# Hxyou/MSCLIP

Hardware: AMD Instinct MI355X
Metric: image-text pairs/sec ViT-B/32 bf16 (higher is better)
Workload: dtype bf16; 1 GPU; MS-CLIP-S b32-yfcc-msclips fwd + contrastive step (both towers, gather, logits, symmetric CE), per-GPU batch 512, 224x224 images + 77-token captions, random-init weights; per_gpu_batch=512, global_batch=512, parallelism=dp1, bn=eval (folded running statistics), rccl_ranks=1

## Files before the change

msclip_amd/csrc/backward.hip:

```cpp
#include <mutex>
#include <type_traits>
#include <stdlib.h>
#include "common.h"
#include "plan.h"
#include "../../include/msclip_hip.h"
#include "../../include/msclip_ext2.h"

namespace {

__device__ __forceinline__ float sigmoidf_fast(float z) { return 1.f / (1.f + __expf(-z)); }

__global__ __launch_bounds__(256) void transpose_kernel(const bf16_t* __restrict__ in, int ldi, bf16_t* __restrict__ out,
                                                        int ldo, int M, int C, int Mpad) {
  __shared__ bf16_t tile[64][66];
  const int m0 = blockIdx.x * 64, c0 = blockIdx.y * 64;
  const int tx = threadIdx.x & 63, ty = threadIdx.x >> 6;
  for (int r = ty; r < 64; r += 4) {
    const int m = m0 + r, c = c0 + tx;
    tile[r][tx] = (m < M && c < C) ? in[(size_t)m * ldi + c] : (bf16_t)0;
  }
  __syncthreads();
  for (int r = ty; r < 64; r += 4) {
    const int c = c0 + r, m = m0 + tx;
    if (c < C && m < Mpad) out[(size_t)c * ldo + m] = tile[tx][r];
// ... 678 lines not shown
                                                int part_blocks, int skip_group, const float* row_scale, void* stream) {
  MSCLIP_PLAN_HOOK(msclip_cast_bf16_colsum_rowscale, stream, x, ldx, y, ldy, M, C, part, part_blocks, skip_group, row_scale);
  return cast_bf16_colsum_launch(x, ldx, y, ldy, M, C, part, part_blocks, skip_group, row_scale, stream);
}

extern "C" int msclip_ext2_abi_version(void) { return MSCLIP_EXT2_ABI_VERSION; }

static bool colsum_two_stage() {
  static int v = -1;
  if (v < 0) {
    const char* e = getenv("MSCLIP_COLSUM_TWO_STAGE");
    v = e && e[0] == '1';
  }
  return v != 0;
}
static unsigned* colsum_counters(int n) {
  constexpr int RING = 1 << 18, MAXDEV = 16;
  static unsigned* ring[MAXDEV] = {};
  static int next[MAXDEV] = {};
  static std::mutex mu;
  int dev = 0;
  if (hipGetDevice(&dev) != hipSuccess || dev < 0 || dev >= MAXDEV || n > RING) return nullptr;
  std::lock_guard<std::mutex> lock(mu);
  if (!ring[dev]) {
    if (hipMalloc((void**)&ring[dev], RING * sizeof(unsigned)) != hipSuccess) { ring[dev] = nullptr; return nullptr; }
    if (hipMemset(ring[dev], 0, RING * sizeof(unsigned)) != hipSuccess || hipDeviceSynchronize() != hipSuccess) return nullptr;
  }
  if (next[dev] + n > RING) next[dev] = 0;
  unsigned* p = ring[dev] + next[dev];
  next[dev] += n;
  return p;
}

extern "C" int msclip_prepare_device(void) { return colsum_counters(0) ? MSCLIP_OK : MSCLIP_ELAUNCH; }

extern "C" int msclip_colsum(const void* x, int ld, int is_f32, float* out, int M, int N, int accumulate, float* scratch,
                             int chunks, void* stream) {
  MSCLIP_PLAN_HOOK(msclip_colsum, stream, x, ld, is_f32, out, M, N, accumulate, scratch, chunks);
  if (!x || !out || M <= 0 || N <= 0 || ld < N || chunks < 1 || (chunks > 1 && !scratch)) return MSCLIP_EINVAL;
  hipStream_t st = (hipStream_t)stream;
  if (is_f32 && M <= 32 && N >= 16384 && !(N % 4) && !(ld % 4) && !((size_t)x % 16) && !((size_t)out % 16)) {
    hipLaunchKernelGGL(fold_rows_kernel, dim3(grid_for((size_t)N / 4, 256, 8192)), dim3(256), 0, st, (const float*)x, (size_t)ld,
                       out, M, (size_t)N / 4, accumulate);
    return msclip_launch_status();
  }
  const int rpc = (M + chunks - 1) / chunks;
  float* first = chunks > 1 ? scratch : out;
  int cpr = 1;
  while (cpr < 32 && cpr * 8 < N) cpr *= 2;
  const bool wide = !is_f32 && !(N % 8) && !(ld % 8) && !((size_t)x % 16);
  const int colblocks = wide ? (N + cpr * 8 - 1) / (cpr * 8) : (N + 63) / 64;
  unsigned* counters = chunks > 1 && !colsum_two_stage() ? colsum_counters(colblocks) : nullptr;
  if (is_f32)
    hipLaunchKernelGGL(colsum_kernel<float>, dim3(colblocks, chunks), dim3(256), 0, st, (const float*)x, ld, first, M, N,
                       chunks > 1 ? 0 : accumulate, rpc, out, counters, accumulate);
  else if (wide)
    hipLaunchKernelGGL(colsum_bf16x8_kernel, dim3(colblocks, chunks), dim3(256), 0, st, (const bf16_t*)x,
                       ld, first, M, N, chunks > 1 ? 0 : accumulate, rpc, cpr, out, counters, accumulate);
  else
    hipLaunchKernelGGL(colsum_kernel<bf16_t>, dim3(colblocks, chunks), dim3(256), 0, st, (const bf16_t*)x, ld, first, M,
                       N, chunks > 1 ? 0 : accumulate, rpc, out, counters, accumulate);
  if (chunks > 1 && !counters)
    hipLaunchKernelGGL(colsum_kernel<float>, dim3((N + 63) / 64, 1), dim3(256), 0, st, (const float*)scratch, N, out, chunks, N,
                       accumulate, chunks);
  return msclip_launch_status();
}

// ... 124 lines not shown
```

msclip_amd/csrc/gemm.hip:

```cpp
#include <stdlib.h>
#include <type_traits>
#include "common.h"
#include "plan.h"
#include "../../include/msclip_hip.h"
#include "../../include/msclip_ext2.h"
#include "gemm_epilogue.h"

namespace {

constexpr int BK = 64;

struct RowSrc {
  long long pix;
  int ih0, iw0;
  int ok;
};



template <int MODE, int BM, int BN, int WM, int WN, bool RS = false>
__global__ __launch_bounds__(WM * WN * 64, 2) void gemm_kernel(const msclip_gemm_desc a_in) {
  msclip_gemm_desc a = a_in;
  if (MODE == 0 && gridDim.y > 1) {
    const int kc = a.K / (int)gridDim.y;
    a.X = (const bf16_t*)a.X + (size_t)blockIdx.y * kc;
    a.W = (const bf16_t*)a.W + (size_t)blockIdx.y * kc;
    a.out = (float*)a.out + (size_t)blockIdx.y * a.M * a.ldo;
    a.K = kc;
  }
  constexpr int NW = WM * WN;
  constexpr int NT = NW * 64;
  constexpr int TM = BM / WM / 32, TN = BN / WN / 32;
  constexpr int XI = BM * 8 / NT, WI = BN * 8 / NT;
  constexpr int NPC = XI + WI;
// ... 179 lines not shown
    else
      epilogue_generic<TM, TN, RS>(acc, a, vec, cm0 + wm, cn0 + wn, lane);
  }
}


constexpr int PSLOTS = 10, PREG = 128 * 64;
#ifndef PP_NOEPI
#define PP_NOEPI 0
#endif

__device__ __forceinline__ bf16x8 pp_ld(const void* p) { return *(const bf16x8*)p; }

typedef __attribute__((ext_vector_type(8))) int i32x8;
template <bool F8>
__device__ __forceinline__ f32x4 pp_mma(const bf16x8 (&w)[2], const bf16x8 (&x)[2], int ks, f32x4 c) {
  if constexpr (F8) {
    i32x8 a, b;
    __builtin_memcpy(&a, &w[0], 32);
    __builtin_memcpy(&b, &x[0], 32);
    return __builtin_amdgcn_mfma_scale_f32_16x16x128_f8f6f4(a, b, c, 0, 0, 0, 0x7f7f7f7f, 0, 0x7f7f7f7f);
  } else {
    return __builtin_amdgcn_mfma_f32_16x16x32_bf16(w[ks], x[ks], c, 0, 0, 0);
  }
}

typedef __attribute__((ext_vector_type(4))) __bf16 bf16x4v;
__device__ __forceinline__ bf16x8 pp_ld_tr(const char* p) {
  const bf16x4v lo = __builtin_amdgcn_ds_read_tr16_b64_v4bf16((AS3 bf16x4v*)p);
  const bf16x4v hi = __builtin_amdgcn_ds_read_tr16_b64_v4bf16((AS3 bf16x4v*)(p + 1024));
  return __builtin_shufflevector(lo, hi, 0, 1, 2, 3, 4, 5, 6, 7);
}

template <int MODE, bool F8 = false, int EPI = 0, bool TNL = false>
__global__ __launch_bounds__(512) void gemm_pp_kernel(const msclip_gemm_desc a_in, const float* __restrict__ row_scale,
                                                      const float* __restrict__ col_scale) {
  static_assert(!(F8 && MODE == 1), "fp8 operands: dense GEMM only");
  static_assert(EPI == 0 || (MODE == 0 && (!F8 || EPI == 2)), "LayerNorm fold: dense GEMM; fp8 operands as the producer only");
  static_assert(EPI != 3 || !F8, "training dgrad epilogue: bf16 operands");
  static_assert(EPI != 4 || !F8, "row-scaled residual update (msclip_gemm_rowscale; row_scale = its table): bf16 operands");
  static_assert(!TNL || (MODE == 0 && !F8 && EPI == 0), "token-major operands: dense bf16 GEMM, plain epilogues");
  msclip_gemm_desc a = a_in;
  if (a.M_dev) a.M = min(a.M, *a.M_dev);
  unsigned kbase = 0;
  const int ktot = a.K;
  if (TNL) {
    const int kc = ((a.K + 63) / 64 + (int)gridDim.y - 1) / (int)gridDim.y * 64;
    kbase = blockIdx.y * (unsigned)kc;
    a.out = (float*)a.out + (size_t)blockIdx.y * a.M * a.ldo;
    a.K = kc;
  } else
  if (MODE == 0 && !F8 && gridDim.y > 1) {
    const int kc = a.K / (int)gridDim.y;
    a.X = (const bf16_t*)a.X + (size_t)blockIdx.y * kc;
    a.W = (const bf16_t*)a.W + (size_t)blockIdx.y * kc;
    a.out = (float*)a.out + (size_t)blockIdx.y * a.M * a.ldo;
    a.K = kc;
  }
  constexpr unsigned ES = F8 ? 1u : 2u;
  constexpr int KT = F8 ? 128 : 64;
  constexpr int TM = 4, TN = 2;
  constexpr bool TE = MODE == 0 && !F8 && EPI == 0;
  __shared__ __attribute__((aligned(1024))) bf16_t smem[PSLOTS * PREG];

  const int tid = threadIdx.x;
  const int lane = tid & 63;
  const int wave = __builtin_amdgcn_readfirstlane(tid >> 6);
  const int grp = wave >> 2;
  const int nt_n = (a.N + 255) / 256;
  const int nt_m = (a.M + 255) / 256;
  const int ntiles = nt_n * nt_m;
  const int nk = a.K / KT;

  constexpr int CG = 4;
  const unsigned tper = (unsigned)(nt_m * CG);
  const unsigned tper_rcp = 0xffffffffu / tper + 1u;
  const int wg_tail = nt_n - (nt_n - 1) / CG * CG;
  const unsigned wgt_rcp = 0xffffffffu / (unsigned)wg_tail + 1u;
  auto tile_origin = [&](int t, int& m0, int& n0) {
    const int q = ntiles >> 3, r = ntiles & 7, x = t & 7;
    const unsigned id = (unsigned)((x < r ? x * (q + 1) : r * (q + 1) + (x - r) * q) + (t >> 3));
    const unsigned g = (unsigned)(((unsigned long long)id * tper_rcp) >> 32);
    const unsigned idg = id - g * tper;
    const bool tail = (int)(g * CG + CG) > nt_n;
    const unsigned wg = tail ? (unsigned)wg_tail : (unsigned)CG;
    const unsigned row = !tail ? idg >> 2 : wg_tail == 1 ? idg : (unsigned)(((unsigned long long)idg * wgt_rcp) >> 32);
    m0 = (int)(row * 256u);
    n0 = (int)((g * CG + (idg - row * wg)) * 256u);
  };

  unsigned vx[2], vw[2];
#pragma unroll
  for (int i = 0; i < 2; ++i) {
    if (TNL) {
      const int row = (wave + 8 * i) * 4 + (lane >> 4);
      const int g = (row & 3) | (((row >> 3) & 1) << 2);
      const unsigned ch = (unsigned)(((((lane & 15) >> 1) ^ g) << 1) | (lane & 1)) << 4;
      vx[i] = (unsigned)row * (unsigned)a.ldx * 2u + ch;
      vw[i] = (unsigned)row * (unsigned)a.ldw * 2u + ch;
      continue;
    }
    const int row = (wave + 8 * i) * 8 + (lane >> 3);
    const unsigned ch = (unsigned)((lane & 7) ^ ((row >> 1) & 7)) << 4;
    vx[i] = (unsigned)row * (unsigned)a.ldx * ES + ch;
    vw[i] = (unsigned)row * (unsigned)a.ldw * ES + ch;
  }
  const unsigned xhalf = TNL ? 256u : 128u * (unsigned)a.ldx * ES, whalf = TNL ? 256u : 128u * (unsigned)a.ldw * ES;
  int ti = blockIdx.x, kti = 0, islot = 0;
  __amdgpu_buffer_rsrc_t rx, rw;
  int cpix[2][2], chw[2][2];
  int ce = 0;
  auto set_tile = [&](int t) {
    if (MODE == 1) {
      int m0 = 0, n0 = 0;
      if (t < ntiles) tile_origin(t, m0, n0);
      const int hw = a.Ho * a.Wo;
#pragma unroll
      for (int h = 0; h < 2; ++h)
#pragma unroll
        for (int i = 0; i < 2; ++i) {
          const int row = (wave + 8 * i) * 8 + (lane >> 3);
          const int m = m0 + h * 128 + row;
          const int b = m / hw, rem = m - b * hw;
          const int ho = rem / a.Wo, wo = rem - ho * a.Wo;
          const int ih0 = ho * a.stride - a.pad, iw0 = wo * a.stride - a.pad;
          const int ihs = (t < ntiles && m < a.M) ? ih0 : -(1 << 14);
          chw[h][i] = (ihs & 0xffff) | (iw0 << 16);
          cpix[h][i] = (((b * a.H + ih0) * a.Wd + iw0) * a.Cin) * 2 + (((lane & 7) ^ ((row >> 1) & 7)) << 4);
        }
      const unsigned long long wb = (unsigned long long)(a.N - n0) * (unsigned long long)a.ldw * ES;
      rw = t < ntiles ? make_rsrc((const char*)a.W + (size_t)n0 * a.ldw * ES, wb > 0xffffffffull ? 0xffffffffu : (unsigned)wb)
                      : make_rsrc(a.W, 0);
      return;
    }
    if (TNL) {
      int m0 = 0, n0 = 0;
      if (t < ntiles) tile_origin(t, m0, n0);
      const unsigned long long xb = (unsigned long long)ktot * a.ldx * 2ull - (unsigned long long)m0 * 2ull;
      const unsigned long long wb = (unsigned long long)ktot * a.ldw * 2ull - (unsigned long long)n0 * 2ull;
      rx = t < ntiles ? make_rsrc((const char*)a.X + (size_t)m0 * 2, (unsigned)xb) : make_rsrc(a.X, 0);
      rw = t < ntiles ? make_rsrc((const char*)a.W + (size_t)n0 * 2, (unsigned)wb) : make_rsrc(a.W, 0);
// ... 19 lines not shown
    if (TNL) {
      const unsigned kr = kbase + (unsigned)kti * 64u;
      if (J < 2) {
        const unsigned ro = kr * (unsigned)a.ldw * 2u;
        blds16(rw, vw[0] + ro, (J & 1) * 256u, dst);
        blds16(rw, vw[1] + ro, (J & 1) * 256u, dst + 8 * 512);
      } else {
        const unsigned ro = kr * (unsigned)a.ldx * 2u;
        blds16(rx, vx[0] + ro, (J & 1) * 256u, dst);
        blds16(rx, vx[1] + ro, (J & 1) * 256u, dst + 8 * 512);
      }
    } else
    if (J < 2) {
      blds16(rw, vw[0], ko + (J & 1) * whalf, dst);
      blds16(rw, vw[1], ko + (J & 1) * whalf, dst + 8 * 512);
    } else if (MODE == 1) {
      const int kh = (ce >> 20) & 15, kw = (ce >> 24) & 15, doff = (ce & 0xfffff) * 2;
#pragma unroll
      for (int i = 0; i < 2; ++i) {
        const int ih = ((chw[J & 1][i] << 16) >> 16) + kh, iw = (chw[J & 1][i] >> 16) + kw;
        const bool ok = (unsigned)ih < (unsigned)a.H && (unsigned)iw < (unsigned)a.Wd;
        blds16(rx, ok ? (unsigned)(cpix[J & 1][i] + doff) : 0x80000000u, 0, dst + i * 8 * 512);
      }
    } else {
      blds16(rx, vx[0], ko + (J & 1) * xhalf, dst);
      blds16(rx, vx[1], ko + (J & 1) * xhalf, dst + 8 * 512);
    }
    if (MODE == 1 && J == 1) {
      const int* tp = a.ktab + kti * 8;
      asm volatile("s_load_dword %0, %1, 0x0\n\ts_waitcnt lgkmcnt(0)" : "=s"(ce) : "s"(tp));
    }
    islot = islot == PSLOTS - 1 ? 0 : islot + 1;
    if (J == 3) {
      if (++kti == nk) {
        kti = 0;
        ti += gridDim.x;
        set_tile(ti);
      }
    }
  };
  using I0 = std::integral_constant<int, 0>;
  using I1 = std::integral_constant<int, 1>;
  using I2 = std::integral_constant<int, 2>;
  using I3 = std::integral_constant<int, 3>;

  const int wm = grp * 128, wn = (wave & 3) * 64;
  const int r16 = lane & 15, quad = lane >> 4;
  const bool vec = !((a.N | a.ldo | (a.resid_kind ? a.ldr : 0)) & 3);
  const bool plain_rows = a.rpg == 0x7fffffff && a.resid_kind != 3 && a.resid_kind < 5;
  int la[2];
#pragma unroll
  for (int ks = 0; ks < 2; ++ks)
    la[ks] = r16 * 128 + (((F8 ? (quad << 1) | ks : (ks << 2) | quad) ^ ((r16 >> 1) & 7)) << 4);
  const int wsub = ((wave >> 1) & 1);
  const int woff = (wave & 1) * 64 * 128;
  const int lt = (8 * quad + (r16 >> 2)) * 256 + ((((r16 >> 2) & 3) | ((quad & 1) << 2)) << 5) + (r16 & 3) * 8;
  const int ltw = lt ^ ((wave & 1) * 128);
  const char* lds = (const char*)smem;

  if (MODE == 1)
    rx = make_rsrc(a.X, (unsigned)((long long)(a.M / (a.Ho * a.Wo)) * a.H * a.Wd * a.Cin * 2));
  set_tile(ti);
  issue(I0{}); issue(I1{}); issue(I2{}); issue(I3{});
  issue(I0{}); issue(I1{}); issue(I2{});
  issue(I3{});
  asm volatile("s_waitcnt vmcnt(8)" ::: "memory");
  __builtin_amdgcn_s_barrier();
  asm volatile("" ::: "memory");
  if (grp) __builtin_amdgcn_s_barrier();

  int cslot = 0;
  bf16x8 w0[2][2], w1[2][2], xf[4][2];
  int epi_stores = 0;
  for (int tc = blockIdx.x; tc < ntiles; tc += gridDim.x) {
    int cm0, cn0;
    tile_origin(tc, cm0, cn0);
    f32x4 acc[4][8];
#pragma unroll
    for (int i = 0; i < 4; ++i)
#pragma unroll
      for (int j = 0; j < 8; ++j)
#pragma unroll
        for (int r = 0; r < 4; ++r) acc[i][j][r] = 0.f;
    int lane_s;
    asm volatile("v_mbcnt_lo_u32_b32 %0, -1, 0\n\tv_mbcnt_hi_u32_b32 %0, -1, %0" : "=v"(lane_s));
    const bool seg2 = EPI == 1 && a.W2 && cm0 >= a.seg_split;
    const float* bseg = seg2 ? a.bias2 : a.bias;
    const float* bsrc = bseg ? bseg : (const float*)a.zero;
    const int nlast = bseg ? a.N - 1 : 0;
    float bcol;
    {
      const int n = cn0 + wn + lane_s;
      const float* p = bsrc + (n < nlast ? n : nlast);
      asm volatile("global_load_dword %0, %1, off" : "=&v"(bcol) : "v"(p));
    }
    float ccol = 0.f;
    f32x4 rstat4 = {1.f, 0.f, 1.f, 0.f};
    if constexpr (EPI == 1) {
      const float* p = (seg2 ? a.csum2 : a.csum) + cn0 + wn + lane_s;
      asm volatile("global_load_dword %0, %1, off" : "=&v"(ccol) : "v"(p));
      const float* q0 = a.rowstat + 2 * (size_t)(cm0 + wm + lane_s);
      f32x2 lo, hi;
      asm volatile("global_load_dwordx2 %0, %1, off" : "=&v"(lo) : "v"(q0));
      asm volatile("global_load_dwordx2 %0, %1, off offset:512" : "=&v"(hi) : "v"(q0));
      rstat4 = f32x4{lo[0], lo[1], hi[0], hi[1]};
    } else if constexpr (EPI == 2) {
      const float* q0 = a.center + cm0 + wm + lane_s;
      float lo, hi;
      asm volatile("global_load_dword %0, %1, off" : "=&v"(lo) : "v"(q0));
      asm volatile("global_load_dword %0, %1, off offset:256" : "=&v"(hi) : "v"(q0));
      rstat4 = f32x4{lo, 0.f, hi, 0.f};
    }

    float pf_sink = 0.f;
    for (int kt = 0; kt < nk; ++kt) {
      int s1 = cslot + wsub, s2 = cslot + 2 + grp;
      if (s1 >= PSLOTS) s1 -= PSLOTS;
      if (s2 >= PSLOTS) s2 -= PSLOTS;
      const char* wreg = lds + s1 * (PREG * 2) + woff;
      const char* xreg = lds + s2 * (PREG * 2);
      cslot = cslot + 4 >= PSLOTS ? cslot + 4 - PSLOTS : cslot + 4;

#define PP_PRIO(x) __builtin_amdgcn_s_setprio(x)
#define PP_LGK() asm volatile("s_waitcnt lgkmcnt(0)" ::: "memory")
#define PP_SYNC_IN()                                   \
  __builtin_amdgcn_sched_barrier(0);                   \
  __builtin_amdgcn_s_barrier();                        \
  PP_LGK();                                            \
  __builtin_amdgcn_sched_barrier(0);                   \
  PP_PRIO(1)
#define PP_SYNC_OUT()                                  \
  PP_PRIO(0);                                          \
  __builtin_amdgcn_sched_barrier(0);                   \
  __builtin_amdgcn_s_barrier();                        \
  asm volatile("" ::: "memory");                       \
  __builtin_amdgcn_sched_barrier(0)

      const size_t wtn = (size_t)(lds + s1 * (PREG * 2) + ltw), xtn = (size_t)(lds + s2 * (PREG * 2) + lt);
      if constexpr (TNL) {
#pragma unroll
        for (int i = 0; i < 2; ++i)
#pragma unroll
          for (int ks = 0; ks < 2; ++ks) w0[i][ks] = pp_ld_tr((const char*)(wtn ^ (size_t)(i * 32)) + ks * 8192);
        __builtin_amdgcn_sched_barrier(0);
#pragma unroll
        for (int j = 0; j < 4; ++j)
#pragma unroll
          for (int ks = 0; ks < 2; ++ks) xf[j][ks] = pp_ld_tr((const char*)(xtn ^ (size_t)(j * 32)) + ks * 8192);
// ... 27 lines not shown
        for (int j = 0; j < 4; ++j)
#pragma unroll
          for (int i = 0; i < 2; ++i)
            acc[i][j] = pp_mma<F8>(w0[i], xf[j], ks, acc[i][j]);
#pragma unroll
      for (int ks = 0; ks < (F8 ? 1 : 2); ++ks)
#pragma unroll
        for (int j = 0; j < 4; ++j)
#pragma unroll
          for (int i = 0; i < 2; ++i)
            acc[2 + i][j] = pp_mma<F8>(w1[i], xf[j], ks, acc[2 + i][j]);
      PP_SYNC_OUT();

      if constexpr (TNL) {
#pragma unroll
        for (int j = 0; j < 4; ++j)
#pragma unroll
          for (int ks = 0; ks < 2; ++ks) xf[j][ks] = pp_ld_tr((const char*)(xtn ^ (size_t)((4 + j) * 32)) + ks * 8192);
      } else {
#pragma unroll
      for (int j = 0; j < 4; ++j)
#pragma unroll
        for (int ks = 0; ks < 2; ++ks) xf[j][ks] = pp_ld(xreg + 8192 + j * 2048 + la[ks]);
      }
      if (!kt) {
        issue(I0{});
        issue(I1{});
      }
      issue(I2{});
      issue(I3{});
      if constexpr (EPI == 1 || EPI == 2) {
        if (kt == 2) {
          int nm0, nn0;
          tile_origin(tc + (int)gridDim.x < ntiles ? tc + (int)gridDim.x : tc, nm0, nn0);
          const float* q = (EPI == 1 ? a.rowstat + 2 * (size_t)(nm0 + wm) : a.center + (nm0 + wm)) + (lane_s & (EPI == 1 ? 7 : 3)) * 32;
          asm volatile("global_load_dword %0, %1, off" : "=&v"(pf_sink) : "v"(q));
        }
      }
      if ((EPI == 1 || EPI == 2) && kt == 2) asm volatile("s_waitcnt vmcnt(9)" ::: "memory");
      else
      if (kt == 0 && nk >= 3 && epi_stores == 16) asm volatile("s_waitcnt vmcnt(24)" ::: "memory");
      else if (kt == 0 && nk >= 3 && epi_stores == 32) asm volatile("s_waitcnt vmcnt(40)" ::: "memory");
      else if (EPI == 3 && kt == 0 && nk >= 3 && epi_stores == 34) asm volatile("s_waitcnt vmcnt(42)" ::: "memory");
      else if (kt == 0 && nk >= 3 && epi_stores == 52) asm volatile("s_waitcnt vmcnt(60)" ::: "memory");
      else asm volatile("s_waitcnt vmcnt(8)" ::: "memory");
      PP_SYNC_IN();
#pragma unroll
      for (int ks = 0; ks < (F8 ? 1 : 2); ++ks)
#pragma unroll
        for (int j = 0; j < 4; ++j)
#pragma unroll
          for (int i = 0; i < 2; ++i)
            acc[2 + i][4 + j] = pp_mma<F8>(w1[i], xf[j], ks, acc[2 + i][4 + j]);

#pragma unroll
      for (int ks = 0; ks < (F8 ? 1 : 2); ++ks)
#pragma unroll
        for (int j = 0; j < 4; ++j)
#pragma unroll
          for (int i = 0; i < 2; ++i)
            acc[i][4 + j] = pp_mma<F8>(w0[i], xf[j], ks, acc[i][4 + j]);
      PP_SYNC_OUT();
    }

    if (!grp) __builtin_amdgcn_s_barrier();
    asm volatile("" : "+v"(pf_sink)::"memory");
    {
      int ss = cslot + 8 + (wave >> 2);
      while (ss >= PSLOTS) ss -= PSLOTS;
      const unsigned stg = (unsigned)(size_t)(AS3 bf16_t*)smem + ss * (PREG * 2) + (wave & 3) * STG_BYTES;
      int lane_e;
      asm volatile("v_mbcnt_lo_u32_b32 %0, -1, 0\n\tv_mbcnt_hi_u32_b32 %0, -1, %0" : "=v"(lane_e));
      epi_stores = 0;
#if PP_NOEPI
      {
        float sacc = 0.f;
#pragma unroll
        for (int i = 0; i < 4; ++i)
#pragma unroll
          for (int j = 0; j < 8; ++j) sacc += (acc[i][j][0] + acc[i][j][1]) + (acc[i][j][2] + acc[i][j][3]);
        if (sacc == 1.2345678e-30f) ((float*)a.zero)[lane_e] = sacc;
      }
#else
      if (F8) {
        const int er = lane_e & 15, eq = lane_e >> 4;
#pragma unroll
        for (int mi = 0; mi < 8; ++mi) {
          const int m = cm0 + wm + mi * 16 + er;
          const float sx = row_scale[m < a.M ? m : a.M - 1];
#pragma unroll
          for (int ni = 0; ni < 4; ++ni)
#pragma unroll
            for (int r = 0; r < 4; ++r) acc[ni][mi][r] *= sx;
        }
#pragma unroll
        for (int ni = 0; ni < 4; ++ni)
#pragma unroll
          for (int r = 0; r < 4; ++r) {
            const int n = cn0 + wn + ni * 16 + eq * 4 + r;
            const float sw = col_scale[n < a.N ? n : a.N - 1];
#pragma unroll
            for (int mi = 0; mi < 8; ++mi) acc[ni][mi][r] *= sw;
          }
      }
      if constexpr (EPI == 1) {
        const float4 rstat = make_float4(rstat4[0], rstat4[1], rstat4[2], rstat4[3]);
// ... 16 lines not shown
          epilogue_rows<TM, TN, 1, 0, 1, false, true>(acc, a, stg, cm0 + wm, cn0 + wn, lane_e, bcol, row_scale);
        } else {
          epilogue_generic16<TM, TN, true>(acc, a, vec, cm0 + wm, cn0 + wn, lane_e, row_scale);
        }
      } else
      if (vec && plain_rows && cm0 + 256 <= a.M)
      {
        const bool full_n = cn0 + 256 <= a.N;
        const int mw0 = cm0 + wm, nw0 = cn0 + wn;
        const bool pack16 = a.resid_kind == 0 && a.out_kind == 0 && !((a.N | a.ldo) & 7);
        if (F8 && a.out_kind == 2) {
          if (full_n) epi_stores = 2 * TM;
          if (a.act == 1) epilogue_pack8<TM, TN, 1>(acc, a, stg, mw0, nw0, lane_e, bcol, a.out_scale);
          else epilogue_pack8<TM, TN, 0>(acc, a, stg, mw0, nw0, lane_e, bcol, a.out_scale);
        } else {
        if (full_n) epi_stores = pack16 && a.act <= 2 ? (a.out2 ? 8 * TM : 4 * TM) : 4 * TM * TN;
        if (TE && pack16 && a.out2)
          epilogue_pack16<TM, TN, 0>(acc, a, stg, mw0, nw0, lane_e, bcol, a.out2);
        if (pack16 && a.act == 0)
          epilogue_pack16<TM, TN, 0>(acc, a, stg, mw0, nw0, lane_e, bcol, a.out);
        else if (pack16 && a.act == 1)
          epilogue_pack16<TM, TN, 1>(acc, a, stg, mw0, nw0, lane_e, bcol, a.out);
        else if (pack16 && a.act == 2)
          epilogue_pack16<TM, TN, 2>(acc, a, stg, mw0, nw0, lane_e, bcol, a.out);
        else if (a.resid_kind == 1 && a.act == 0 && a.out_kind == 1)
          epilogue_rows<TM, TN, 1, 0, 1>(acc, a, stg, mw0, nw0, lane_e, bcol);
        else
          epilogue_rows<TM, TN, -1, -1, -1>(acc, a, stg, mw0, nw0, lane_e, bcol);
        }
      }
      else
        epilogue_generic16<TM, TN>(acc, a, vec, cm0 + wm, cn0 + wn, lane_e);
#endif
    }
    if (grp) __builtin_amdgcn_s_barrier();
    asm volatile("" ::: "memory");
  }
  asm volatile("s_waitcnt vmcnt(0)" ::: "memory");
#undef PP_SYNC_IN
#undef PP_SYNC_OUT
#undef PP_PRIO
#undef PP_LGK
}

}

template <int MODE, int BM, int BN, int WM, int WN>
static void launch_cfg(const msclip_gemm_desc* d, hipStream_t st, int blocks_per_cu) {
  const int ncu = msclip_device_cus();
  const int tiles = ((d->M + BM - 1) / BM) * ((d->N + BN - 1) / BN);
  const int cap = ncu * blocks_per_cu;
  const int grid = tiles < cap ? tiles : cap;
  hipLaunchKernelGGL((gemm_kernel<MODE, BM, BN, WM, WN>), dim3(grid), dim3(WM * WN * 64), 0, st, *d);
}

template <int BM, int BN, int WM, int WN>
static void launch_cfg_rowscale(const msclip_gemm_desc* d, hipStream_t st, int blocks_per_cu, const float* rscale) {
  const int ncu = msclip_device_cus();
  const int tiles = ((d->M + BM - 1) / BM) * ((d->N + BN - 1) / BN);
  const int cap = ncu * blocks_per_cu;
  const int grid = tiles < cap ? tiles : cap;
  msclip_gemm_desc d2 = *d;
  d2.csum = rscale;
  hipLaunchKernelGGL((gemm_kernel<0, BM, BN, WM, WN, true>), dim3(grid), dim3(WM * WN * 64), 0, st, d2);
}

// ... 46 lines not shown
  if ((d->tile == 0 || d->tile == 5) && !train_epi && !fold_c && !fold_p && msclip_gemm_small_eligible(d)) return GV_STREAM;
  if (d->mode == 0) {
    const bool pp_ok = (long long)d->ldx * 2 * 256 + (long long)d->K * 2 < (1ll << 31) &&
                       (long long)d->ldw * 2 * 256 + (long long)d->K * 2 < (1ll << 31) &&
                       big_tiles * ((d->M + 255) / 256) * 4 < (1ll << 32);
    if (pp_ok && d->resid_kind < 5 && (d->tile == 4 || (d->tile == 0 && big))) return GV_PP;
    if (train_epi || fold_c || fold_p) return GV_INVALID;
    if (d->tile == 6) return GV_DENSE192;
    return GV_DENSE128;
  }
  const long long in_bytes = (long long)(d->M / (d->Ho * d->Wo)) * d->H * d->Wd * d->Cin * 2;
  if ((d->tile == 0 || d->tile == 4) && d->Cin % 64 == 0 && d->K % d->Cin == 0 && in_bytes < (1ll << 31) &&
      (long long)d->ldw * 2 * 256 + (long long)d->K * 2 < (1ll << 31) && d->rpg == 0x7fffffff && d->resid_kind != 3 &&
      d->resid_kind < 5 && d->M % (d->Ho * d->Wo) == 0 && (big_tiles >= 128 || d->tile == 4) && big_tiles * ((d->M + 255) / 256) * 4 < (1ll << 32))
    return GV_PPCONV;
  const long long t192 = (long long)((d->M + 255) / 256) * ((d->N + 191) / 192);
  if (d->tile == 6 || (d->tile == 0 && d->N % 192 == 0 && t192 >= 128)) return GV_CONV192;
  return GV_CONV128;
}

extern "C" const char* msclip_gemm_variant(const msclip_gemm_desc* d) { return kVariantName[pick_variant(d)]; }

extern "C" int msclip_gemm_splitk(const msclip_gemm_desc* d, int slices, void* stream) {
  MSCLIP_PLAN_HOOK(msclip_gemm_splitk, stream, d, slices);
  if (!d || slices < 1 || slices > 65535 || pick_variant(d) == GV_INVALID || d->M_dev) return MSCLIP_EINVAL;
  if (d->mode != 0 || d->out_kind != 1 || d->bias || d->resid || d->resid_kind || d->act || d->rpg != 0x7fffffff || d->radd ||
      d->roff || (d->K % (BK * slices)))
    return MSCLIP_EINVAL;
  if (d->tile == 4) {
    if (pick_variant(d) != GV_PP) return MSCLIP_EINVAL;
    const int t256 = ((d->M + 255) / 256) * ((d->N + 255) / 256);
    const int ncu = device_cus();
    hipLaunchKernelGGL((gemm_pp_kernel<0, false>), dim3(t256 < ncu ? t256 : ncu, slices), dim3(512), 0, (hipStream_t)stream, *d,
                       nullptr, nullptr);
    return msclip_launch_status();
  }
  const int tiles = ((d->M + 127) / 128) * ((d->N + 127) / 128);
  const int cap = device_cus() * 2;
  hipLaunchKernelGGL((gemm_kernel<0, 128, 128, 2, 2>), dim3(tiles < cap ? tiles : cap, slices), dim3(256), 0,
                     (hipStream_t)stream, *d);
  return msclip_launch_status();
}

extern "C" int msclip_gemm_splitk_tn(const msclip_gemm_desc* d, int slices, void* stream) {
  MSCLIP_PLAN_HOOK(msclip_gemm_splitk_tn, stream, d, slices);
  if (!d || !d->X || !d->W || !d->out || !d->zero || slices < 1 || slices > 65535 || d->M_dev) return MSCLIP_EINVAL;
  if (d->M <= 0 || d->N <= 0 || d->K <= 0 || (d->ldx % 8) || (d->ldw % 8) || d->ldx < d->M || d->ldw < d->N || (d->ldo % 4) ||
      d->ldo < d->N || d->mode != 0 || d->out_kind != 1 || d->bias || d->resid || d->resid_kind || d->act || d->out2 || d->xb ||
      d->rowstat || d->W2 || d->rpg != 0x7fffffff || d->radd || d->roff || d->alpha != 1.f)
    return MSCLIP_EINVAL;
  const long long t256 = (long long)((d->M + 255) / 256) * ((d->N + 255) / 256);
  const long long krows = ((long long)d->K + 63) / 64 * 64 + 64ll * (slices + 1);
  if (krows * d->ldx * 2 + 4096 >= (1ll << 32) || krows * d->ldw * 2 + 4096 >= (1ll << 32) ||
      t256 * ((d->M + 255) / 256) * 4 >= (1ll << 32))
    return MSCLIP_EINVAL;
  const int ncu = device_cus();
  hipLaunchKernelGGL((gemm_pp_kernel<0, false, 0, true>), dim3(t256 < ncu ? (int)t256 : ncu, slices), dim3(512), 0,
                     (hipStream_t)stream, *d, nullptr, nullptr);
  return msclip_launch_status();
}

extern "C" int msclip_gemm_f8(const msclip_gemm_desc* d, const float* row_scale, const float* col_scale, void* stream) {
  MSCLIP_PLAN_HOOK(msclip_gemm_f8, stream, d, row_scale, col_scale);
  if (!d || !d->X || !d->W || !d->out || !d->zero || !row_scale || !col_scale) return MSCLIP_EINVAL;
  if (d->mode != 0 || d->M <= 0 || d->N <= 0 || d->K <= 0 || (d->K % 128) || (d->ldx % 16) || (d->ldw % 16) || d->ldx < d->K ||
      d->ldw < d->K || d->rpg != 0x7fffffff || d->out2 || d->out_kind < 0 || d->out_kind > 2 || d->resid_kind < 0 || d->resid_kind > 2 ||
      d->rowstat || d->W2)
    return MSCLIP_EINVAL;
  if (d->out_kind == 2 && ((d->M % 256) || (d->N % 16) || (d->ldo % 16) || d->resid_kind || !(d->out_scale > 0.f)))
    return MSCLIP_EINVAL;
  const long long tiles = (long long)((d->M + 255) / 256) * ((d->N + 255) / 256);
  if ((long long)d->ldx * 256 + d->K >= (1ll << 31) || (long long)d->ldw * 256 + d->K >= (1ll << 31) ||
      tiles * ((d->M + 255) / 256) * 4 >= (1ll << 32))
    return MSCLIP_EINVAL;
  const int ncu = device_cus();
  if (d->xb) {
    if (d->resid_kind != 1 || d->out_kind != 1 || d->act || !d->center || !d->part || (d->M % 256) || (d->N % 256) || (d->ldxb % 4) ||
        (d->ldo % 4) || (d->ldr % 4) || (d->resid2 && (d->seg_split <= 0 || (d->seg_split % 256) || d->seg_split >= d->M)))
      return MSCLIP_EINVAL;
    hipLaunchKernelGGL((gemm_pp_kernel<0, true, 2>), dim3(tiles < ncu ? (int)tiles : ncu), dim3(512), 0, (hipStream_t)stream, *d,
                       row_scale, col_scale);
    return msclip_launch_status();
  }
  hipLaunchKernelGGL((gemm_pp_kernel<0, true>), dim3(tiles < ncu ? (int)tiles : ncu), dim3(512), 0, (hipStream_t)stream, *d,
                     row_scale, col_scale);
  return msclip_launch_status();
}

extern "C" int msclip_gemm(const msclip_gemm_desc* d, void* stream) {
  MSCLIP_PLAN_HOOK(msclip_gemm, stream, d);
  const GemmVariant v = pick_variant(d);
  if (v == GV_INVALID) return MSCLIP_EINVAL;
  if (d->M_dev && v != GV_PP) return MSCLIP_EINVAL;
  hipStream_t st = (hipStream_t)stream;
  const int ncu = device_cus();
  const int tiles = ((d->M + 255) / 256) * ((d->N + 255) / 256);
  const int grid = tiles < ncu ? tiles : ncu;
  switch (v) {
    case GV_STREAM: if (!msclip_gemm_small_try(d, st, ncu)) return MSCLIP_EINVAL; break;
    case GV_PP:
      if (d->rowstat) hipLaunchKernelGGL((gemm_pp_kernel<0, false, 1>), dim3(grid), dim3(512), 0, st, *d, nullptr, nullptr);
      else if (d->xb) hipLaunchKernelGGL((gemm_pp_kernel<0, false, 2>), dim3(grid), dim3(512), 0, st, *d, nullptr, nullptr);
      else if (d->resid_kind == 4) hipLaunchKernelGGL((gemm_pp_kernel<0, false, 3>), dim3(grid), dim3(512), 0, st, *d, nullptr, nullptr);
      else hipLaunchKernelGGL((gemm_pp_kernel<0, false>), dim3(grid), dim3(512), 0, st, *d, nullptr, nullptr);
      break;
    case GV_PPCONV: hipLaunchKernelGGL((gemm_pp_kernel<1, false>), dim3(grid), dim3(512), 0, st, *d, nullptr, nullptr); break;
    case GV_DENSE128:
      if (!msclip_gemm_skinny_try(d, st, ncu)) launch_cfg<0, 128, 128, 2, 2>(d, st, 2);
      break;
    case GV_CONV192: launch_cfg<1, 256, 192, 4, 2>(d, st, 1); break;
    case GV_DENSE192: launch_cfg<0, 256, 192, 4, 2>(d, st, 1); break;
    case GV_CONV128: launch_cfg<1, 128, 128, 2, 2>(d, st, 2); break;
    default: return MSCLIP_EINVAL;
  }
  return msclip_launch_status();
}

extern "C" int msclip_gemm_rowscale(const msclip_gemm_desc* d, const float* row_scale, void* stream) {
  if (!row_scale) return msclip_gemm(d, stream);
  MSCLIP_PLAN_HOOK(msclip_gemm_rowscale, stream, d, row_scale);
  const GemmVariant v = pick_variant(d);
  if (v == GV_INVALID) return MSCLIP_EINVAL;
  if (d->mode != 0 || d->resid_kind != 1 || !d->resid || d->out_kind != 1 || d->act || d->out2 || d->xb || d->rowstat || d->W2 ||
      d->part || d->bn_mode || d->resid2)
    return MSCLIP_EINVAL;
  if (d->M_dev && v != GV_PP) return MSCLIP_EINVAL;
  hipStream_t st = (hipStream_t)stream;
  const int ncu = device_cus();
  const int tiles = ((d->M + 255) / 256) * ((d->N + 255) / 256);
  const int grid = tiles < ncu ? tiles : ncu;
  switch (v) {
    case GV_PP: hipLaunchKernelGGL((gemm_pp_kernel<0, false, 4>), dim3(grid), dim3(512), 0, st, *d, row_scale, nullptr); break;
    case GV_STREAM:
      if (d->tile != 0) return MSCLIP_EINVAL;
      launch_cfg_rowscale<128, 128, 2, 2>(d, st, 2, row_scale);
      break;
    case GV_DENSE128: launch_cfg_rowscale<128, 128, 2, 2>(d, st, 2, row_scale); break;
    case GV_DENSE192: launch_cfg_rowscale<256, 192, 4, 2>(d, st, 1, row_scale); break;
    default: return MSCLIP_EINVAL;
  }
  return msclip_launch_status();
}
```

Before: 51030 pairs/s.

## Split-K the tail wave of persistent PP GEMM across idle CUs

When the tile count leaves a small remainder wave on the persistent GEMM grid, the leftover tiles are split along K into up to four slices. Each slice writes fp32 partials to a global workspace, and an atomic counter elects the last block to sum them and run the epilogue. This targets idle CUs during the final partial wave. In exchange it adds workspace allocation, atomics and extra global traffic for the partial sums. It is on by default via an environment flag and only applies when K is large enough.

```diff
diff --git a/msclip_amd/csrc/backward.hip b/msclip_amd/csrc/backward.hip
--- a/msclip_amd/csrc/backward.hip
+++ b/msclip_amd/csrc/backward.hip
@@ -734,7 +734,11 @@
   return p;
 }
 
-extern "C" int msclip_prepare_device(void) { return colsum_counters(0) ? MSCLIP_OK : MSCLIP_ELAUNCH; }
+int msclip_gemm_tail_prepare();
+extern "C" int msclip_prepare_device(void) {
+  if (!colsum_counters(0)) return MSCLIP_ELAUNCH;
+  return msclip_gemm_tail_prepare();
+}
 
 extern "C" int msclip_colsum(const void* x, int ld, int is_f32, float* out, int M, int N, int accumulate, float* scratch,
                              int chunks, void* stream) {
diff --git a/msclip_amd/csrc/gemm.hip b/msclip_amd/csrc/gemm.hip
--- a/msclip_amd/csrc/gemm.hip
+++ b/msclip_amd/csrc/gemm.hip
@@ -1,5 +1,7 @@
 #include <stdlib.h>
+#include <mutex>
 #include <type_traits>
+#include <vector>
 #include "common.h"
 #include "plan.h"
 #include "../../include/msclip_hip.h"
@@ -245,9 +247,19 @@
   return __builtin_shufflevector(lo, hi, 0, 1, 2, 3, 4, 5, 6, 7);
 }
 
+constexpr int PP_TAIL_CNT_BYTES = 4096;
+constexpr int PP_TAIL_SLAB_F4 = 256 * 256 / 4;
+__host__ __device__ inline int pp_tail_slices(int ntiles, int G, int nk, int min_nks) {
+  const int r = ntiles % G;
+  if (ntiles < G || r == 0 || 2 * r > G) return 1;
+  for (int s = 4; s >= 2; --s)
+    if (nk % s == 0 && nk / s >= min_nks && r * s <= G) return s;
+  return 1;
+}
+
 template <int MODE, bool F8 = false, int EPI = 0, bool TNL = false>
 __global__ __launch_bounds__(512) void gemm_pp_kernel(const msclip_gemm_desc a_in, const float* __restrict__ row_scale,
-                                                      const float* __restrict__ col_scale) {
+                                                      const float* __restrict__ col_scale, unsigned* __restrict__ tail_ws, int tail_min_nks) {
   static_assert(!(F8 && MODE == 1), "fp8 operands: dense GEMM only");
   static_assert(EPI == 0 || (MODE == 0 && (!F8 || EPI == 2)), "LayerNorm fold: dense GEMM; fp8 operands as the producer only");
   static_assert(EPI != 3 || !F8, "training dgrad epilogue: bf16 operands");
@@ -274,6 +286,7 @@
   constexpr int KT = F8 ? 128 : 64;
   constexpr int TM = 4, TN = 2;
   constexpr bool TE = MODE == 0 && !F8 && EPI == 0;
+  constexpr bool SPL = MODE == 0 && !F8 && !TNL && (EPI == 0 || EPI == 2);
   __shared__ __attribute__((aligned(1024))) bf16_t smem[PSLOTS * PREG];
 
   const int tid = threadIdx.x;
@@ -284,6 +297,23 @@
   const int nt_m = (a.M + 255) / 256;
   const int ntiles = nt_n * nt_m;
   const int nk = a.K / KT;
+  const int G = (int)gridDim.x;
+  int F = ntiles, nitems = ntiles, nks = nk;
+  int tail_tile = 0, tail_k0 = 0, tail_S = 1;
+  if (SPL && tail_ws) {
+    const int S = pp_tail_slices(ntiles, G, nk, tail_min_nks);
+    if (S > 1) {
+      const int R = ntiles % G;
+      F = ntiles - R;
+      nitems = F + R * S;
+      nks = nk / S;
+      tail_S = S;
+      const int q = (int)(((unsigned)blockIdx.x * (65536u / (unsigned)S + 1u)) >> 16);
+      tail_tile = F + q;
+      tail_k0 = ((int)blockIdx.x - q * S) * nks;
+    }
+  }
+  auto item_tile = [&](int i) { return !SPL || i < F ? i : i < nitems ? tail_tile : ntiles; };
 
   constexpr int CG = 4;
   const unsigned tper = (unsigned)(nt_m * CG);
@@ -320,6 +350,7 @@
   }
   const unsigned xhalf = TNL ? 256u : 128u * (unsigned)a.ldx * ES, whalf = TNL ? 256u : 128u * (unsigned)a.ldw * ES;
   int ti = blockIdx.x, kti = 0, islot = 0;
+  int kend = nk;
   __amdgpu_buffer_rsrc_t rx, rw;
   int cpix[2][2], chw[2][2];
   int ce = 0;
@@ -405,10 +436,14 @@
     }
     islot = islot == PSLOTS - 1 ? 0 : islot + 1;
     if (J == 3) {
-      if (++kti == nk) {
+      if (++kti == kend) {
         kti = 0;
         ti += gridDim.x;
-        set_tile(ti);
+        if (SPL && ti >= F && ti < nitems) {
+          kti = tail_k0;
+          kend = tail_k0 + nks;
+        }
+        set_tile(item_tile(ti));
       }
     }
   };
@@ -433,7 +468,7 @@
 
   if (MODE == 1)
     rx = make_rsrc(a.X, (unsigned)((long long)(a.M / (a.Ho * a.Wo)) * a.H * a.Wd * a.Cin * 2));
-  set_tile(ti);
+  set_tile(item_tile(ti));
   issue(I0{}); issue(I1{}); issue(I2{}); issue(I3{});
   issue(I0{}); issue(I1{}); issue(I2{});
   issue(I3{});
@@ -445,7 +480,10 @@
   int cslot = 0;
   bf16x8 w0[2][2], w1[2][2], xf[4][2];
   int epi_stores = 0;
-  for (int tc = blockIdx.x; tc < ntiles; tc += gridDim.x) {
+  for (int ic = blockIdx.x; ic < nitems; ic += gridDim.x) {
+    const int tc = item_tile(ic);
+    const bool slice = SPL && ic >= F;
+    const int nkc = slice ? nks : nk;
     int cm0, cn0;
     tile_origin(tc, cm0, cn0);
     f32x4 acc[4][8];
@@ -486,7 +524,7 @@
     }
 
     float pf_sink = 0.f;
-    for (int kt = 0; kt < nk; ++kt) {
+    for (int kt = 0; kt < nkc; ++kt) {
       int s1 = cslot + wsub, s2 = cslot + 2 + grp;
       if (s1 >= PSLOTS) s1 -= PSLOTS;
       if (s2 >= PSLOTS) s2 -= PSLOTS;
@@ -580,17 +618,17 @@
       if constexpr (EPI == 1 || EPI == 2) {
         if (kt == 2) {
           int nm0, nn0;
-          tile_origin(tc + (int)gridDim.x < ntiles ? tc + (int)gridDim.x : tc, nm0, nn0);
+          tile_origin(ic + (int)gridDim.x < nitems ? item_tile(ic + (int)gridDim.x) : tc, nm0, nn0);
           const float* q = (EPI == 1 ? a.rowstat + 2 * (size_t)(nm0 + wm) : a.center + (nm0 + wm)) + (lane_s & (EPI == 1 ? 7 : 3)) * 32;
           asm volatile("global_load_dword %0, %1, off" : "=&v"(pf_sink) : "v"(q));
         }
       }
       if ((EPI == 1 || EPI == 2) && kt == 2) asm volatile("s_waitcnt vmcnt(9)" ::: "memory");
       else
-      if (kt == 0 && nk >= 3 && epi_stores == 16) asm volatile("s_waitcnt vmcnt(24)" ::: "memory");
-      else if (kt == 0 && nk >= 3 && epi_stores == 32) asm volatile("s_waitcnt vmcnt(40)" ::: "memory");
-      else if (EPI == 3 && kt == 0 && nk >= 3 && epi_stores == 34) asm volatile("s_waitcnt vmcnt(42)" ::: "memory");
-      else if (kt == 0 && nk >= 3 && epi_stores == 52) asm volatile("s_waitcnt vmcnt(60)" ::: "memory");
+      if (kt == 0 && nkc >= 3 && epi_stores == 16) asm volatile("s_waitcnt vmcnt(24)" ::: "memory");
+      else if (kt == 0 && nkc >= 3 && epi_stores == 32) asm volatile("s_waitcnt vmcnt(40)" ::: "memory");
+      else if (EPI == 3 && kt == 0 && nkc >= 3 && epi_stores == 34) asm volatile("s_waitcnt vmcnt(42)" ::: "memory");
+      else if (kt == 0 && nkc >= 3 && epi_stores == 52) asm volatile("s_waitcnt vmcnt(60)" ::: "memory");
       else asm volatile("s_waitcnt vmcnt(8)" ::: "memory");
       PP_SYNC_IN();
 #pragma unroll
@@ -620,6 +658,57 @@
       int lane_e;
       asm volatile("v_mbcnt_lo_u32_b32 %0, -1, 0\n\tv_mbcnt_hi_u32_b32 %0, -1, %0" : "=v"(lane_e));
       epi_stores = 0;
+      bool run_epi = true;
+      if constexpr (SPL) {
+        if (slice) {
+          typedef __attribute__((ext_vector_type(4))) float slab4;
+          const int tid_e = wave * 64 + lane_e;
+          slab4* slabs = (slab4*)((char*)tail_ws + PP_TAIL_CNT_BYTES);
+          slab4* mine = slabs + (size_t)blockIdx.x * PP_TAIL_SLAB_F4 + tid_e;
+#pragma unroll
+          for (int i = 0; i < 4; ++i)
+#pragma unroll
+            for (int j = 0; j < 8; ++j) mine[(i * 8 + j) * 512] = acc[i][j];
+          __builtin_amdgcn_s_waitcnt(0x0f70);
+          asm volatile("" ::: "memory");
+          __syncthreads();
+          unsigned* flag = (unsigned*)(smem + cslot * PREG);
+          if (wave == 0 && lane_e == 0) {
+            __builtin_amdgcn_fence(__ATOMIC_RELEASE, "agent");
+            asm volatile("s_waitcnt vmcnt(0)" ::: "memory");
+            const unsigned tk = __hip_atomic_fetch_add(tail_ws + (tail_tile - F), 1u, __ATOMIC_RELAXED, __HIP_MEMORY_SCOPE_AGENT);
+            if (tk == (unsigned)(tail_S - 1)) {
+              __hip_atomic_store(tail_ws + (tail_tile - F), 0u, __ATOMIC_RELAXED, __HIP_MEMORY_SCOPE_AGENT);
+              __builtin_amdgcn_fence(__ATOMIC_ACQUIRE, "agent");
+              asm volatile("s_waitcnt vmcnt(0)" ::: "memory");
+            }
+            *flag = tk;
+          }
+          __syncthreads();
+          run_epi = *flag == (unsigned)(tail_S - 1);
+          if (run_epi) {
+            const slab4* sl = slabs + (size_t)(tail_tile - F) * tail_S * PP_TAIL_SLAB_F4 + tid_e;
+#pragma unroll
+            for (int i = 0; i < 4; ++i)
+#pragma unroll
+              for (int j = 0; j < 8; ++j) acc[i][j] = f32x4{0.f, 0.f, 0.f, 0.f};
+            for (int s = 0; s < tail_S; ++s, sl += PP_TAIL_SLAB_F4) {
+#pragma unroll
+              for (int h = 0; h < 2; ++h) {
+                slab4 t[16];
+#pragma unroll
+                for (int e = 0; e < 16; ++e) t[e] = sl[(h * 16 + e) * 512];
+                __builtin_amdgcn_sched_barrier(0);
+#pragma unroll
+                for (int e = 0; e < 16; ++e) acc[h * 2 + e / 8][e % 8] += t[e];
+                __builtin_amdgcn_sched_barrier(0);
+              }
+            }
+            __builtin_amdgcn_s_waitcnt(0x0f70);
+          }
+        }
+      }
+      if (run_epi) {
 #if PP_NOEPI
       {
         float sacc = 0.f;
@@ -702,6 +791,7 @@
       else
         epilogue_generic16<TM, TN>(acc, a, vec, cm0 + wm, cn0 + wn, lane_e);
 #endif
+      }
     }
     if (grp) __builtin_amdgcn_s_barrier();
     asm volatile("" ::: "memory");
@@ -814,7 +904,7 @@
     const int t256 = ((d->M + 255) / 256) * ((d->N + 255) / 256);
     const int ncu = device_cus();
     hipLaunchKernelGGL((gemm_pp_kernel<0, false>), dim3(t256 < ncu ? t256 : ncu, slices), dim3(512), 0, (hipStream_t)stream, *d,
-                       nullptr, nullptr);
+                       nullptr, nullptr, nullptr, 0);
     return msclip_launch_status();
   }
   const int tiles = ((d->M + 127) / 128) * ((d->N + 127) / 128);
@@ -838,7 +928,7 @@
     return MSCLIP_EINVAL;
   const int ncu = device_cus();
   hipLaunchKernelGGL((gemm_pp_kernel<0, false, 0, true>), dim3(t256 < ncu ? (int)t256 : ncu, slices), dim3(512), 0,
-                     (hipStream_t)stream, *d, nullptr, nullptr);
+                     (hipStream_t)stream, *d, nullptr, nullptr, nullptr, 0);
   return msclip_launch_status();
 }
 
@@ -861,12 +951,90 @@
         (d->ldo % 4) || (d->ldr % 4) || (d->resid2 && (d->seg_split <= 0 || (d->seg_split % 256) || d->seg_split >= d->M)))
       return MSCLIP_EINVAL;
     hipLaunchKernelGGL((gemm_pp_kernel<0, true, 2>), dim3(tiles < ncu ? (int)tiles : ncu), dim3(512), 0, (hipStream_t)stream, *d,
-                       row_scale, col_scale);
+                       row_scale, col_scale, nullptr, 0);
     return msclip_launch_status();
   }
   hipLaunchKernelGGL((gemm_pp_kernel<0, true>), dim3(tiles < ncu ? (int)tiles : ncu), dim3(512), 0, (hipStream_t)stream, *d,
-                     row_scale, col_scale);
+                     row_scale, col_scale, nullptr, 0);
   return msclip_launch_status();
+}
+
+static bool tail_split_enabled() {
+  static int v = -1;
+  if (v < 0) {
+    const char* e = getenv("MSCLIP_GEMM_TAIL_SPLIT");
+    v = !(e && e[0] == '0');
+  }
+  return v != 0;
+}
+static int tail_min_nks() {
+  static int v = -1;
+  if (v < 0) {
+    const char* e = getenv("MSCLIP_GEMM_TAIL_MIN_NKS");
+    v = e ? atoi(e) : 12;
+    if (v < 2) v = 2;
+  }
+  return v;
+}
+struct TailRegion { int dev; bool owned; hipStream_t st; unsigned* base; };
+static std::vector<TailRegion> g_tail_regions;
+static std::mutex g_tail_mu;
+constexpr int kTailSpares = 4;
+static unsigned* tail_region_alloc(int ncu) {
+  unsigned* p = nullptr;
+  if (hipMalloc((void**)&p, (size_t)PP_TAIL_CNT_BYTES + (size_t)ncu * PP_TAIL_SLAB_F4 * 16) != hipSuccess) {
+    (void)hipGetLastError();
+    return nullptr;
+  }
+  return p;
+}
+static unsigned* tail_region(hipStream_t st, int ncu) {
+  const int dev = msclip_dev_index();
+  if (dev < 0) return nullptr;
+  std::lock_guard<std::mutex> lock(g_tail_mu);
+  for (const TailRegion& r : g_tail_regions)
+    if (r.owned && r.dev == dev && r.st == st) return r.base;
+  hipStreamCaptureStatus cs = hipStreamCaptureStatusNone;
+  if (hipStreamIsCapturing(st, &cs) != hipSuccess) {
+    (void)hipGetLastError();
+    return nullptr;
+  }
+  if (cs == hipStreamCaptureStatusNone) {
+    unsigned* p = tail_region_alloc(ncu);
+    if (p && hipMemsetAsync(p, 0, PP_TAIL_CNT_BYTES, st) != hipSuccess) {
+      (void)hipGetLastError();
+      return nullptr;
+    }
+    if (p) g_tail_regions.push_back(TailRegion{dev, true, st, p});
+    return p;
+  }
+  for (TailRegion& r : g_tail_regions)
+    if (!r.owned && r.dev == dev) {
+      r.owned = true;
+      r.st = st;
+      return r.base;
+    }
+  return nullptr;
+}
+int msclip_gemm_tail_prepare() {
+  if (!tail_split_enabled()) return MSCLIP_OK;
+  const int dev = msclip_dev_index();
+  if (dev < 0) return MSCLIP_OK;
+  std::lock_guard<std::mutex> lock(g_tail_mu);
+  int have = 0;
+  for (const TailRegion& r : g_tail_regions) have += !r.owned && r.dev == dev;
+  for (; have < kTailSpares; ++have) {
+    unsigned* p = tail_region_alloc(device_cus());
+    if (!p || hipMemset(p, 0, PP_TAIL_CNT_BYTES) != hipSuccess || hipDeviceSynchronize() != hipSuccess) return MSCLIP_ELAUNCH;
+    g_tail_regions.push_back(TailRegion{dev, false, nullptr, p});
+  }
+  return MSCLIP_OK;
+}
+static unsigned* tail_ws_for(const msclip_gemm_desc* d, hipStream_t st, int tiles, int ncu) {
+  if (!tail_split_enabled() || tiles <= ncu || d->resid_kind == 4 || d->rowstat) return nullptr;
+  if (d->K / 64 < 2 * tail_min_nks()) return nullptr;
+  if (!d->M_dev && pp_tail_slices(tiles, ncu, d->K / 64, tail_min_nks()) == 1) return nullptr;
+  return tail_region(st, ncu);
 }
 
 extern "C" int msclip_gemm(const msclip_gemm_desc* d, void* stream) {
@@ -880,13 +1048,15 @@
   const int grid = tiles < ncu ? tiles : ncu;
   switch (v) {
     case GV_STREAM: if (!msclip_gemm_small_try(d, st, ncu)) return MSCLIP_EINVAL; break;
-    case GV_PP:
-      if (d->rowstat) hipLaunchKernelGGL((gemm_pp_kernel<0, false, 1>), dim3(grid), dim3(512), 0, st, *d, nullptr, nullptr);
-      else if (d->xb) hipLaunchKernelGGL((gemm_pp_kernel<0, false, 2>), dim3(grid), dim3(512), 0, st, *d, nullptr, nullptr);
-      else if (d->resid_kind == 4) hipLaunchKernelGGL((gemm_pp_kernel<0, false, 3>), dim3(grid), dim3(512), 0, st, *d, nullptr, nullptr);
-      else hipLaunchKernelGGL((gemm_pp_kernel<0, false>), dim3(grid), dim3(512), 0, st, *d, nullptr, nullptr);
+    case GV_PP: {
+      unsigned* tw = tail_ws_for(d, st, tiles, ncu);
+      if (d->rowstat) hipLaunchKernelGGL((gemm_pp_kernel<0, false, 1>), dim3(grid), dim3(512), 0, st, *d, nullptr, nullptr, nullptr, 0);
+      else if (d->xb) hipLaunchKernelGGL((gemm_pp_kernel<0, false, 2>), dim3(grid), dim3(512), 0, st, *d, nullptr, nullptr, tw, tail_min_nks());
+      else if (d->resid_kind == 4) hipLaunchKernelGGL((gemm_pp_kernel<0, false, 3>), dim3(grid), dim3(512), 0, st, *d, nullptr, nullptr, nullptr, 0);
+      else hipLaunchKernelGGL((gemm_pp_kernel<0, false>), dim3(grid), dim3(512), 0, st, *d, nullptr, nullptr, tw, tail_min_nks());
       break;
-    case GV_PPCONV: hipLaunchKernelGGL((gemm_pp_kernel<1, false>), dim3(grid), dim3(512), 0, st, *d, nullptr, nullptr); break;
+    }
+    case GV_PPCONV: hipLaunchKernelGGL((gemm_pp_kernel<1, false>), dim3(grid), dim3(512), 0, st, *d, nullptr, nullptr, nullptr, 0); break;
     case GV_DENSE128:
       if (!msclip_gemm_skinny_try(d, st, ncu)) launch_cfg<0, 128, 128, 2, 2>(d, st, 2);
       break;
@@ -912,7 +1082,7 @@
   const int tiles = ((d->M + 255) / 256) * ((d->N + 255) / 256);
   const int grid = tiles < ncu ? tiles : ncu;
   switch (v) {
-    case GV_PP: hipLaunchKernelGGL((gemm_pp_kernel<0, false, 4>), dim3(grid), dim3(512), 0, st, *d, row_scale, nullptr); break;
+    case GV_PP: hipLaunchKernelGGL((gemm_pp_kernel<0, false, 4>), dim3(grid), dim3(512), 0, st, *d, row_scale, nullptr, nullptr, 0); break;
     case GV_STREAM:
       if (d->tile != 0) return MSCLIP_EINVAL;
       launch_cfg_rowscale<128, 128, 2, 2>(d, st, 2, row_scale);
```

New measurement: 51090 pairs/s, median of 4. No clear change (+0.1%).
